# AniruddhaMandal/SS-GNN

Measured on AMD Instinct MI355X. Metric: k_subgraphs_sampled_per_sec, higher is better.
Workload: dtype int64; 1 GPU; c5_er_1m; graphs=1, columns=19999981, k=8, rows_per_gpu=1000000, global_rows=1000000, mode=sample, collate=none (single GPU)

## Files before the change

### ss-gnn_amd/csrc/ugs_kernels.hip

```cpp
#include "ugs_device.h"
#include <cstdlib>

#define UGS_ALIGNED16 __attribute__((aligned(16)))

#ifdef UGS_STAMPS
__device__ unsigned long long ugs_stamp_buffer[32];
#define ST_ ws.ST
#define STAMP_DECL unsigned long long st_t0 = 0
#define STAMP_BEGIN() do { __builtin_amdgcn_sched_barrier(0); st_t0 = __builtin_amdgcn_s_memtime(); __builtin_amdgcn_sched_barrier(0); } while (0)
#define STAMP_END(i) do { __builtin_amdgcn_sched_barrier(0); const unsigned long long t1_ = __builtin_amdgcn_s_memtime(); \
    if ((threadIdx.x & 63) == 0) { atomicAdd(&ST_[i], t1_ - st_t0); atomicAdd(&ST_[16 + (i)], 1ull); } st_t0 = __builtin_amdgcn_s_memtime(); __builtin_amdgcn_sched_barrier(0); } while (0)
#define STAMP_SUB_BEGIN() __builtin_amdgcn_sched_barrier(0); const unsigned long long sti_ = __builtin_amdgcn_s_memtime(); __builtin_amdgcn_sched_barrier(0)
#define STAMP_SUB_END_OF(parent, i) do { __builtin_amdgcn_sched_barrier(0); const unsigned long long t1_ = __builtin_amdgcn_s_memtime(); \
    if ((threadIdx.x & 63) == 0) { atomicAdd(&ST_[i], t1_ - sti_); atomicAdd(&ST_[parent], sti_ - t1_); atomicAdd(&ST_[16 + (i)], 1ull); } __builtin_amdgcn_sched_barrier(0); } while (0)
#define STAMP_SUB_END(i) STAMP_SUB_END_OF(2, i)
#else
#define STAMP_DECL
#define STAMP_SUB_BEGIN() do {} while (0)
#define STAMP_SUB_END(i) do {} while (0)
#define STAMP_SUB_END_OF(parent, i) do {} while (0)
#define STAMP_BEGIN() do {} while (0)
#define STAMP_END(i) do {} while (0)
#endif

// ... 864 lines not shown
    }
    return fm;
}

#define UGS_NO_ENTRY make_int2(-1, -1)
template <int GS, class SP, bool ADD, bool STG, bool GUARD = true, bool SON = false>
__device__ __forceinline__ bool scan_chunk(const Work<SP> &ws, const Grp<GS> &g, uint32_t v, uint32_t root_vi, uint32_t size, uint32_t &c,
                                           uint32_t &hcount, uint32_t &ecount, StageCtx &sc, int2 e, uint32_t p) {
    const uint32_t w = (uint32_t)e.x;
    const bool cand = e.y >= (int)root_vi;
    uint32_t slot = hash_slot(w, ws.hmask);
    const uint32_t step = hash_step(w);
    bool in_s = false;
    if constexpr (GS == 64 && sizeof(typename SP::TW) == 4) {
        if (ADD) {
            if constexpr (GUARD) { if (hcount + (uint32_t)__popcll(__ballot(cand)) > ws.hlimit) return false; }
            uint32_t seen = kKeyMask;
            STAMP_SUB_BEGIN();
            slot = probe_insert_lds(ws.HK, ws.hmask, slot, step, w, seen, e.y, root_vi);
            STAMP_SUB_END_OF(1, 6);
            const uint64_t insm = __ballot(seen == kEmpty);
            const uint64_t im = __ballot((int)seen < -1);
            const uint64_t dupm = __ballot((int)seen >= (int)kFresh);
            SP::sync();
            uint64_t fm = insm;
            if (__builtin_expect(dupm != 0ull, 0)) fm = first_of_repeated(g, w, insm, dupm);
            if (__builtin_amdgcn_inverse_ballot_w64(insm)) ws.HK[slot] = w;
            ecount += __builtin_amdgcn_inverse_ballot_w64(im) ? (w == v ? 1u : 2u) : 0u;
            if constexpr (STG) stage_hits_mask<SON>(sc, g, im, w, p, size);
            const uint32_t nnew = (uint32_t)__popcll(fm);
            if constexpr (GUARD) { if (c + nnew > ws.cap) return false; }
            if (__builtin_amdgcn_inverse_ballot_w64(fm)) ws.D[c + g.below(fm)] = w;
            c += nnew;
            hcount += nnew;
            SP::sync();
        } else {
            uint32_t seen = kEmpty;
            probe_find_lds(ws.HK, ws.hmask, slot, step, w, seen, e.y, root_vi);
            const uint64_t im = __ballot((int)seen < -1);
            ecount += __builtin_amdgcn_inverse_ballot_w64(im) ? (w == v ? 1u : 2u) : 0u;
            if constexpr (STG) stage_hits_mask<SON>(sc, g, im, w, p, size);
        }
        return true;
    } else
    if (ADD) {
        if constexpr (GUARD) { if (hcount + (uint32_t)__popcll(g.ballot(cand)) > ws.hlimit) return false; }
        uint32_t seen = kKeyMask;
        STAMP_SUB_BEGIN();
        if constexpr (sizeof(typename SP::TW) == 4) {
            slot = probe_insert_lds_v(reinterpret_cast<uint32_t *>(ws.HK), ws.hmask, slot, step, w, seen, e.y, root_vi);
        } else
        if (cand) {
            for (uint32_t it = 0; it <= ws.hmask; ++it) {
                seen = atomicCAS(&ws.HK[slot], kEmpty, w | kFresh);
                if (seen == kEmpty || (seen & kKeyMask) == w) break;
                slot = (slot + step) & ws.hmask;
            }
        }
        STAMP_SUB_END_OF(1, 6);
        const bool inserted = seen == kEmpty;
        in_s = (seen & (kKeyMask | kInS)) == (w | kInS);
        const bool fresh_dup = (seen & (kKeyMask | kFresh)) == (w | kFresh);
        SP::sync();
        bool first = inserted;
        uint64_t dupm = g.ballot(fresh_dup);
        while (dupm) {
            const int li = __ffsll((long long)dupm) - 1;
            const uint32_t wi = g.bcast(w, li);
            const bool mine = cand && w == wi;
            const uint64_t grp = g.ballot(mine);
            if (mine) first = g.lane == (__ffsll((long long)grp) - 1);
            dupm &= ~grp;
        }
        if (inserted) ws.HK[slot] = w;
        if constexpr (GS == 64) ecount += in_s ? (w == v ? 1u : 2u) : 0u;
        else
        {
            const uint64_t im = g.ballot(in_s), sm = g.ballot(w == v);
            ecount += 2u * (uint32_t)__popcll(im & ~sm) + (uint32_t)__popcll(im & sm);
        }
        if constexpr (STG) { if (sc.on) stage_hits<GS>(sc, g, in_s, w, p, size); }
        const uint64_t fm = g.ballot(first);
        const uint32_t nnew = (uint32_t)__popcll(fm);
        if constexpr (GUARD) { if (c + nnew > ws.cap) return false; }
        if (first) ws.D[c + g.below(fm)] = w;
        c += nnew;
        hcount += nnew;
        SP::sync();
    } else {
        uint32_t seen = kEmpty;
        if constexpr (sizeof(typename SP::TW) == 4) {
            probe_find_lds_v(reinterpret_cast<const uint32_t *>(ws.HK), ws.hmask, slot, step, w, seen, e.y, root_vi);
        } else
        if (cand) {
            for (uint32_t it = 0; it <= ws.hmask; ++it) {
                seen = ws.HK[slot];
                if (seen == kEmpty || (seen & kKeyMask) == w) break;
                slot = (slot + step) & ws.hmask;
            }
        }
        in_s = (seen & (kKeyMask | kInS)) == (w | kInS);
        if constexpr (GS == 64) ecount += in_s ? (w == v ? 1u : 2u) : 0u;
        else
        {
            const uint64_t im = g.ballot(in_s), sm = g.ballot(w == v);
            ecount += 2u * (uint32_t)__popcll(im & ~sm) + (uint32_t)__popcll(im & sm);
        }
        if constexpr (STG) { if (sc.on) stage_hits<GS>(sc, g, in_s, w, p, size); }
    }
    return true;
}

constexpr uint32_t kNoMember = 0xFFFFFFFEu;
__device__ __forceinline__ uint32_t last_row_members(const Grp<64> &g, const uint32_t *SV, uint32_t size) {
    return (uint32_t)g.lane < size ? SV[g.lane & (UGS_KMAX - 1)] : kNoMember;
}
template <bool SON>
__device__ __forceinline__ void scan_chunk_last(const Grp<64> &g, uint32_t v, uint32_t size, uint32_t &ecount, StageCtx &sc,
                                                uint32_t w, uint32_t p, uint32_t members) {
    uint64_t im = 0ull;
#pragma unroll
    for (int j = 0; j < 8; ++j) im |= __ballot(w == (uint32_t)__builtin_amdgcn_readlane((int)members, j));
    if (__builtin_expect(size > 8u, 0)) {
        for (uint32_t j = 8; j < size; j += 4) {
#pragma unroll
            for (uint32_t u = 0; u < 4; ++u) im |= __ballot(w == (uint32_t)__builtin_amdgcn_readlane((int)members, (int)(j + u)));
        }
    }
    ecount += __builtin_amdgcn_inverse_ballot_w64(im) ? (w == v ? 1u : 2u) : 0u;
    stage_hits_mask<SON>(sc, g, im, w, p, size);
}

template <int GS, class SP, bool ADD, bool STG, bool LAST = false>
__device__ __forceinline__ bool scan_row(const Work<SP> &ws, const Grp<GS> &g, const int2 *adj, uint32_t v,
                                         uint32_t root_vi, uint32_t size, uint32_t &c, uint32_t &hcount,
                                         uint32_t &ecount, uint32_t r0, uint32_t r1, StageCtx &sc, const uint32_t *SV = nullptr) {
    if constexpr (LAST) {
        static_assert(GS == 64 && STG && !ADD, "the compare form of the last row: one walk per wave, LDS tiers");
        const uint32_t members = last_row_members(g, SV, size);
        for (uint32_t base = r0; base < r1; base += 64) {
            const uint32_t p = base + (uint32_t)g.lane;
            int2 e = UGS_NO_ENTRY;
            if (p < r1) e = adj[p];
            scan_chunk_last<false>(g, v, size, ecount, sc, (uint32_t)e.x, p, members);
        }
        return true;
    }
    for (uint32_t base = r0; base < r1; base += GS) {
        const uint32_t p = base + (uint32_t)g.lane;
        int2 e = UGS_NO_ENTRY;
        if (p < r1) e = adj[p];
        if (!scan_chunk<GS, SP, ADD, STG>(ws, g, v, root_vi, size, c, hcount, ecount, sc, e, p)) return false;
    }
    return true;
}

__device__ __forceinline__ int2 prow_entry(const UgsPlanDev &P, int64_t vrow, int lane) {
    const uint32_t off = (((uint32_t)vrow << P.prow_shift) + (uint32_t)lane) << 3;
    return *reinterpret_cast<const int2 *>(reinterpret_cast<const char *>(P.prow) + off);
}
__device__ __forceinline__ int2 load_prow(const UgsPlanDev &P, int64_t vrow, int lane) {
    int2 e = make_int2(0, 0);
    if (lane < P.prow_first) e = prow_entry(P, vrow, lane);
    return e;
}

template <class SP, bool ADD, bool STG, bool SON = false, bool LAST = false>
__device__ __forceinline__ bool scan_prow(const Work<SP> &ws, const Grp<64> &g, const UgsPlanDev &P, uint32_t v,
                                          uint32_t root_vi, uint32_t size, uint32_t &c, uint32_t &hcount,
                                          uint32_t &ecount, int2 e0, int64_t vrow, StageCtx &sc, const uint32_t *SV = nullptr) {
    const uint32_t deg = g.bcast((uint32_t)e0.x, 0);
    const uint32_t start = g.bcast((uint32_t)e0.y, 0);
    const uint32_t inl = (1u << P.prow_shift) - 1u;
    const uint32_t n0 = deg < inl ? deg : inl;
    if (n0 >= (uint32_t)P.prow_first) {
        if (g.lane >= P.prow_first && g.lane <= (int)n0) e0 = prow_entry(P, vrow, g.lane);
    }
    if ((uint32_t)(g.lane - 1) >= n0) e0 = UGS_NO_ENTRY;
    if constexpr (LAST) {
        static_assert(STG && !ADD, "the compare form of the last row: one walk per wave, LDS tiers");
        const uint32_t members = last_row_members(g, SV, size);
        if (n0) scan_chunk_last<SON>(g, v, size, ecount, sc, (uint32_t)e0.x, start + (uint32_t)g.lane - 1u, members);
        if (__builtin_expect(deg > inl, 0)) {
            const uint32_t r1 = start + deg;
            for (uint32_t base = start + inl; base < r1; base += 64) {
                const uint32_t p = base + (uint32_t)g.lane;
                int2 e = UGS_NO_ENTRY;
                if (p < r1) e = P.adj[p];
                scan_chunk_last<SON>(g, v, size, ecount, sc, (uint32_t)e.x, p, members);
            }
        }
        return true;
    }
    uint32_t n0a = n0, n0b = n0;
    asm volatile("" : "+s"(n0a));
    asm volatile("" : "+s"(n0b));
    if constexpr (ADD) {
        if (__builtin_expect(hcount + deg <= ws.hlimit && c + deg <= ws.cap, 1)) {
            if (n0a) scan_chunk<64, SP, true, STG, false, SON>(ws, g, v, root_vi, size, c, hcount, ecount, sc, e0, start + (uint32_t)g.lane - 1u);
            if (__builtin_expect(deg > inl, 0)) {
                const uint32_t r1 = start + deg;
                for (uint32_t base = start + inl; base < r1; base += 64) {
                    const uint32_t p = base + (uint32_t)g.lane;
                    int2 e = UGS_NO_ENTRY;
                    if (p < r1) e = P.adj[p];
                    scan_chunk<64, SP, true, STG, false, SON>(ws, g, v, root_vi, size, c, hcount, ecount, sc, e, p);
                }
            }
            return true;
        }
    }
    if (n0b && !scan_chunk<64, SP, ADD, STG, true, SON>(ws, g, v, root_vi, size, c, hcount, ecount, sc, e0, start + (uint32_t)g.lane - 1u)) return false;
    if (__builtin_expect(deg > inl, 0)) {
        const uint32_t r1 = start + deg;
        for (uint32_t base = start + inl; base < r1; base += 64) {
            const uint32_t p = base + (uint32_t)g.lane;
            int2 e = UGS_NO_ENTRY;
            if (p < r1) e = P.adj[p];
            if (!scan_chunk<64, SP, ADD, STG, true, SON>(ws, g, v, root_vi, size, c, hcount, ecount, sc, e, p)) return false;
        }
    }
    return true;
}

constexpr uint32_t kFlushFast = 8u;
#define UGS_ROR_LT(R) "v_sub_co_u32_dpp %1, vcc, %2, %2 row_ror:" #R " row_mask:0xf bank_mask:0xf\n\ts_nop 1\n\tv_addc_co_u32_e32 %0, vcc, 0, %0, vcc\n\t"
template <int N> __device__ __forceinline__ uint32_t ror_count_less(uint32_t key) {
    static_assert(N == 7 || N == 15, "half a DPP row or all of it");
    uint32_t n, diff;
    if constexpr (N == 7)
        asm("v_mov_b32 %0, 0\n\ts_nop 0\n\t" UGS_ROR_LT(1) UGS_ROR_LT(2) UGS_ROR_LT(3) UGS_ROR_LT(4) UGS_ROR_LT(5) UGS_ROR_LT(6) UGS_ROR_LT(7)
            : "=&v"(n), "=&v"(diff) : "v"(key) : "vcc");
    else
        asm("v_mov_b32 %0, 0\n\ts_nop 0\n\t" UGS_ROR_LT(1) UGS_ROR_LT(2) UGS_ROR_LT(3) UGS_ROR_LT(4) UGS_ROR_LT(5) UGS_ROR_LT(6) UGS_ROR_LT(7)
            UGS_ROR_LT(8) UGS_ROR_LT(9) UGS_ROR_LT(10) UGS_ROR_LT(11) UGS_ROR_LT(12) UGS_ROR_LT(13) UGS_ROR_LT(14) UGS_ROR_LT(15)
            : "=&v"(n), "=&v"(diff) : "v"(key) : "vcc");
    return n;
}
#undef UGS_ROR_LT
__device__ __forceinline__ uint32_t flush_hit_lane(uint32_t ne, uint32_t lane) { return ne <= kFlushFast ? (lane & 7u) : lane; }
__device__ __forceinline__ bool flush_has_hit(uint32_t ne, uint32_t lane) {
    return ne <= kFlushFast ? (lane < 16u && (lane & 7u) < ne) : lane < ne;
}

__device__ __forceinline__ void stage_flush(uint32_t ne, const Grp<64> &g, const uint32_t *SV, uint32_t k, uint4 en, uint32_t ecol, uint2 *out) {
    const uint32_t lane = (uint32_t)g.lane;
    uint32_t ei = 0u;
    if (k <= 8u) {
        const uint4 s0 = reinterpret_cast<const uint4 *>(SV)[0], s1 = reinterpret_cast<const uint4 *>(SV)[1];
        ei = (s1.w == en.y) ? 7u : ei; ei = (s1.z == en.y) ? 6u : ei; ei = (s1.y == en.y) ? 5u : ei; ei = (s1.x == en.y) ? 4u : ei;
        ei = (s0.w == en.y) ? 3u : ei; ei = (s0.z == en.y) ? 2u : ei; ei = (s0.y == en.y) ? 1u : ei; ei = (s0.x == en.y) ? 0u : ei;
    } else {
        for (uint32_t j = 0; j < k; ++j) ei = (SV[j] == en.y) ? j : ei;
    }
    const uint32_t es = en.z;
    if (__builtin_expect(ne <= kFlushFast, 1)) {
        const bool have = lane < 16u && (lane & 7u) < ne;
        if (__builtin_expect(!g.any(have && ei == es), 1)) {
            const uint32_t col = have ? ecol : 0xFFFFFFFFu;
            const uint32_t cr = ror_count_less<7>(col);
            const bool fwd = lane < 8u;
            const uint32_t src = fwd ? es : ei, dst = fwd ? ei : es;
            const uint32_t key = have ? src * 8u + cr : 0xFFFFFFFFu;
            const uint32_t rank = ror_count_less<15>(key);
            if (have) out[rank] = make_uint2(ecol, src | (dst << 8));
            return;
        }
    }
    const bool mine = lane < ne;
    uint32_t cr = 0u;
    const uint32_t ecol_s = mine ? ecol : 0xFFFFFFFFu;
    if (g.any(mine && ei == es)) {
        for (uint32_t t = 0; t < ne; t += 4) {
#pragma unroll
            for (uint32_t u = 0; u < 4; ++u) {
                const uint32_t ct = g.bcast(ecol_s, (int)((t + u) & 63u));
                cr += (ct < ecol || (ct == ecol && t + u < lane)) ? 1u : 0u;
            }
        }
    } else {
        for (uint32_t t = 0; t < ne; t += 4) {
#pragma unroll
            for (uint32_t u = 0; u < 4; ++u) cr += g.bcast(ecol_s, (int)((t + u) & 63u)) < ecol ? 1u : 0u;
        }
    }
    const bool mirror = mine && ei != es;
    const uint32_t ka = es * UGS_STAGE_ENTRIES + cr, kb = ei * UGS_STAGE_ENTRIES + cr;
    const uint32_t kk = (ka << 16) | kb;
    uint32_t ra = 0u, rb = 0u;
    const uint32_t kk_s = mine ? kk : 0xFFFFFFFFu;
    for (uint32_t t = 0; t < ne; t += 4) {
#pragma unroll
        for (uint32_t u = 0; u < 4; ++u) {
            const uint32_t kt = g.bcast(kk_s, (int)((t + u) & 63u));
            const uint32_t kat = kt >> 16, kbt = ((kt >> 21) == ((kt >> 5) & 0x7FFu)) ? 0xFFFFu : (kt & 0xFFFFu);
            ra += (kat < ka ? 1u : 0u) + (kbt < ka ? 1u : 0u);
            rb += (kat < kb ? 1u : 0u) + (kbt < kb ? 1u : 0u);
        }
    }
    if (mine) out[ra] = make_uint2(ecol, es | (ei << 8));
    if (mirror) out[rb] = make_uint2(ecol, ei | (es << 8));
}

template <int GS, class SP, int MAXPER, bool PAD, bool SEEDS = false, bool UNI = false>
__device__ __forceinline__ bool do_walk(const Work<SP> &ws, const Grp<GS> &g_, const UgsWalkArgs &a, int64_t row_rel,
                                        uint32_t *SV , uint4 *EL ,
                                        uint32_t *nedges_out = nullptr ) {

    static_assert(!PAD || GS == 64, "padded rows are read by a whole wave");
    static_assert(!UNI || (PAD && !SEEDS && sizeof(typename SP::TW) == 4), "UNI: one graph, one seed, padded rows, staging on");
    const Grp<GS> &g = g_;
    constexpr bool STG = GS == 64 && sizeof(typename SP::TW) == 4;
    StageCtx sc;
    sc.EL = EL; sc.ne = 0u; sc.on = STG && a.stage != nullptr && EL != nullptr; sc.onm = 0ull;
    if constexpr (UNI) { sc.on = true; sc.onm = ~0ull; }
    else if constexpr (STG) {
        uint32_t on32 = g.uni(sc.on ? 1u : 0u);
        asm volatile("" : "+s"(on32));
        sc.onm = 0ull - (uint64_t)on32;
    }
    const UgsPlanDev &P = a.plan;
    const int64_t row = a.row_begin + row_rel;
    int64_t gi, i;
    if (UNI || P.num_graphs == 1) { gi = 0; i = row; }
    else { gi = row / a.m; i = row - gi * a.m; }
    const UgsGraphDesc gd = P.graphs[gi];
    const int k = a.k;
    int64_t *out = a.nodes + row_rel * k;
    if (nedges_out) *nedges_out = 0u;
    if (gd.level < 0) {
        for (int j = g.lane; j < k; j += GS) out[j] = -1;
        if (g.lane == 0) a.counts[row_rel] = 0;
        return true;
    }
    STAMP_DECL;
    STAMP_BEGIN();
    Rng rng;
    uint64_t seed_base;
    if constexpr (SEEDS) seed_base = a.seeds[gi];
    else seed_base = a.seed_ptr ? *a.seed_ptr : a.seed64;
    rng.init(seed_base + (uint64_t)i * 0x9e3779b97f4a7c15ull);
    uint32_t root_vi, root_v;
    uint32_t j = 0;
    double u = 0.0;
    UgsRootRec rr{};
    int2 vr = make_int2(0, 0);
    if (gd.level == 0) {
        j = mod64_root(rng.next(), (uint32_t)gd.n);
        u = (double)rng.next() * 0x1p-64;
        rr = P.roots[gd.vbase + j];
    } else {
        const uint32_t idx = mod64_root(rng.next(), (uint32_t)gd.n_viable);
        vr = P.viable[gd.viable_base + idx];
    }
    __builtin_amdgcn_sched_barrier(0);
    {
        uint4 *H4 = reinterpret_cast<uint4 *>(ws.HK);
        const uint32_t n4 = (ws.hmask + 1u) >> 2;
        for (uint32_t s = g.lane; s < n4; s += GS) H4[s] = make_uint4(kEmpty, kEmpty, kEmpty, kEmpty);
    }
    if (gd.level == 0) {
        const bool self = u < rr.prob;
        root_vi = g.uni(self ? j : (uint32_t)rr.alias);
        root_v = g.uni((uint32_t)(self ? rr.v_self : rr.v_alias));
    } else {
        root_vi = g.uni((uint32_t)vr.x);
        root_v = g.uni((uint32_t)vr.y);
    }
    uint32_t r0 = 0, r1 = 0;
    int2 e0 = make_int2(0, 0);
    uint32_t v = root_v;
    if constexpr (PAD) e0 = load_prow(P, gd.vbase + v, g.lane);
    else { r0 = g.uni((uint32_t)P.rowptr[gd.rbase + v]); r1 = g.uni((uint32_t)P.rowptr[gd.rbase + v + 1]); }
    SP::sync();
    if (g.lane == 0) { ws.HK[hash_slot(root_v, ws.hmask)] = root_v | kInS; SV[0] = root_v; }
    SP::sync();
    uint32_t size = 1, c = 0, hcount = 1, ecount = 0;
    int nvalid = 0;
    STAMP_END(0);
    const bool root_only = STG && k == 1;
    bool last_row = root_only;
    for (int step = 0; !root_only; ++step) {
        Grp<GS> g = g_;
        if constexpr (GS == 64) asm volatile("" : "+v"(g.lane));
#ifdef UGS_PAD
        {
            uint32_t pad_;
#if UGS_PAD == 1
#define UGS_PAD1 asm volatile("s_mov_b32 %0, 0" : "=s"(pad_));
#elif UGS_PAD == 2
#define UGS_PAD1 asm volatile("s_mov_b32 %0, 0x12345678" : "=s"(pad_));
#elif UGS_PAD == 3
#define UGS_PAD1 asm volatile("v_mov_b32_e32 %0, 0" : "=v"(pad_));
#elif UGS_PAD == 4
#define UGS_PAD1 asm volatile("v_mov_b32_e64 %0, 0" : "=v"(pad_));
#elif UGS_PAD == 5
#define UGS_PAD1 asm volatile("s_cmp_eq_u32 0, 0\ns_cbranch_scc0 ugs_pad_%=\nugs_pad_%=:" : "=s"(pad_) : : "scc");
#elif UGS_PAD == 6
#define UGS_PAD1 asm volatile("s_branch ugs_pad_%=\nugs_pad_%=:" : "=s"(pad_));
#elif UGS_PAD == 7
#define UGS_PAD1 asm volatile("s_nop 0" : "=s"(pad_));
#elif UGS_PAD == 8
#define UGS_PAD1 asm volatile("s_nop 1" : "=s"(pad_));
#else
#define UGS_PAD1 asm volatile("s_waitcnt lgkmcnt(0)" : "=s"(pad_));
#endif
#define UGS_PAD8 UGS_PAD1 UGS_PAD1 UGS_PAD1 UGS_PAD1 UGS_PAD1 UGS_PAD1 UGS_PAD1 UGS_PAD1
            UGS_PAD8 UGS_PAD8 UGS_PAD8 UGS_PAD8 UGS_PAD8 UGS_PAD8 UGS_PAD8 UGS_PAD8
#undef UGS_PAD8
#undef UGS_PAD1
        }
#endif
        bool ok;
        if constexpr (STG) {
            if constexpr (PAD) ok = scan_prow<SP, true, STG, UNI>(ws, g, P, v, root_vi, size, c, hcount, ecount, e0, gd.vbase + v, sc);
            else ok = scan_row<GS, SP, true, STG>(ws, g, P.adj, v, root_vi, size, c, hcount, ecount, r0, r1, sc);
            STAMP_END(1);
            if (!ok) return false;
            if (c == 0) break;
        } else {
            if (step < k - 1) {
                if constexpr (PAD) ok = scan_prow<SP, true, STG, UNI>(ws, g, P, v, root_vi, size, c, hcount, ecount, e0, gd.vbase + v, sc);
                else ok = scan_row<GS, SP, true, STG>(ws, g, P.adj, v, root_vi, size, c, hcount, ecount, r0, r1, sc);
            } else {
                if constexpr (PAD) ok = scan_prow<SP, false, STG, UNI>(ws, g, P, v, root_vi, size, c, hcount, ecount, e0, gd.vbase + v, sc);
                else ok = scan_row<GS, SP, false, STG>(ws, g, P.adj, v, root_vi, size, c, hcount, ecount, r0, r1, sc);
            }
            STAMP_END(1);
            if (!ok) return false;
            if (step >= k - 1 || c == 0) break;
        }
        const uint32_t rsel = g.uni(mod64_by<sizeof(typename SP::TW) == 4, sizeof(typename SP::TW) == 4 && GS == 64>(rng.next(), c));
        STAMP_END(4);
        const Pick pick = select_any<GS, MAXPER>(ws, g, c, rsel, nvalid);
        const uint32_t w = pick.w;
        if constexpr (PAD) {
            e0 = load_prow(P, gd.vbase + w, g.lane);
        } else {
            r0 = (uint32_t)P.rowptr[gd.rbase + w];
            r1 = (uint32_t)P.rowptr[gd.rbase + w + 1];
            r0 = g.uni(r0); r1 = g.uni(r1);
        }
        STAMP_END(2);
        if constexpr (STG) {
            if (size + 1u == (uint32_t)k) {
                SV[size] = w;
                size += 1;
                v = w;
                SP::sync();
                last_row = true;
                break;
            }
        }
        uint32_t q = pick.q;
        if constexpr (sizeof(typename SP::TW) != 4) {
            for (uint32_t t0 = 0; t0 < c && q == c; t0 += 4 * GS) {
                uint32_t x[4];
#pragma unroll
                for (int u = 0; u < 4; ++u) { const uint32_t t = t0 + u * GS + g.lane; x[u] = (t < c) ? ws.D[t] : kEmpty; }
#pragma unroll
                for (int u = 0; u < 4; ++u) {
                    const uint64_t mk = g.ballot(x[u] == w);
                    if (mk && q == c) q = t0 + u * GS + (uint32_t)(__ffsll((long long)mk) - 1);
                }
            }
        }
        STAMP_END(7);
        for (uint32_t t0 = q; t0 + 1 < c; t0 += 4 * GS) {
            uint32_t x[4];
            if constexpr (sizeof(typename SP::TW) == 4) {
#pragma unroll
                for (int u = 0; u < 4; ++u) x[u] = ws.D[t0 + u * GS + g.lane + 1];
                SP::sync();
                {
                    const uint32_t tb = t0 + (uint32_t)g.lane;
                    constexpr uint32_t last = (uint32_t)(MAXPER * GS) - 1u;
#pragma unroll
                    for (int u = 0; u < 4; ++u) {
                        const uint32_t lim4 = (last - (uint32_t)(u * GS)) * 4u, tb4 = tb * 4u;
                        *reinterpret_cast<uint32_t *>(reinterpret_cast<char *>(ws.D + u * GS) + (tb4 < lim4 ? tb4 : lim4)) = x[u];
                    }
                }
            } else {
#pragma unroll
                for (int u = 0; u < 4; ++u) { const uint32_t t = t0 + u * GS + g.lane; x[u] = (t + 1 < c) ? ws.D[t + 1] : 0u; }
                SP::sync();
#pragma unroll
                for (int u = 0; u < 4; ++u) { const uint32_t t = t0 + u * GS + g.lane; if (t + 1 < c) ws.D[t] = x[u]; }
            }
            SP::sync();
        }
        {
            int keep = 0;
            if constexpr (sizeof(typename SP::TW) == 4) {
                if constexpr (GS == 64) keep = chain_index_below_lanes(q + 1u, g_.chain); else
                keep = chain_index_below<nst_of(MAXPER * GS)>(q + 1u);
                keep = keep < nvalid ? keep : nvalid;
            } else {
                while (keep < nvalid && d_chain.B[keep] <= q) ++keep;
            }
            nvalid = keep;
        }
        c -= 1;
        STAMP_END(8);
        {
            const uint32_t step = hash_step(w);
            if constexpr (GS == 64 && sizeof(typename SP::TW) == 4) {
                uint32_t ls;
                asm("v_mul_u32_u24 %0, %1, %2" : "=v"(ls) : "s"(step), "v"(g.lane));
                uint32_t s = (hash_slot(w, ws.hmask) + ls) & ws.hmask;
                const uint32_t addr = (uint32_t)(uintptr_t)ws.HK + (s << 2);
                uint32_t t;
                uint64_t saved, found;
                asm volatile(
                    "s_mov_b64 %[sv], exec\n"
                    "ds_read_b32 %[t], %[addr]\n"
                    "s_waitcnt lgkmcnt(0)\n"
                    "v_cmpx_eq_u32 %[w], %[t]\n"
                    "ds_write_b32 %[addr], %[wf]\n"
                    "s_mov_b64 %[fd], exec\n"
                    "s_mov_b64 exec, %[sv]\n"
                    : [t] "=&v"(t), [sv] "=&s"(saved), [fd] "=&s"(found)
                    : [addr] "v"(addr), [w] "s"(w), [wf] "v"(w | kInS)
                    : "vcc", "memory");
                if (__builtin_expect(found == 0ull, 0)) {
                    bool hit = false;
                    for (uint32_t it = GS; !g.any(hit) && it <= ws.hmask; it += GS) {
                        s = (s + GS * step) & ws.hmask;
                        hit = ws.HK[s] == w;
                    }
                    if (hit) ws.HK[s] = w | kInS;
                }
            } else {
            uint32_t s = (hash_slot(w, ws.hmask) + (uint32_t)g.lane * step) & ws.hmask;
            bool hit = ws.HK[s] == w;
            for (uint32_t it = GS; __builtin_expect(!g.any(hit), 0) && it <= ws.hmask; it += GS) {
                s = (s + GS * step) & ws.hmask;
                hit = ws.HK[s] == w;
            }
            if (hit) ws.HK[s] = w | kInS;
            }
            if constexpr (GS == 64) SV[size] = w;
            else
            if (g.lane == 0) SV[size] = w;
        }
        size += 1;
        v = w;
        SP::sync();
        STAMP_END(3);
    }
    if constexpr (STG) {
        if (last_row) {
            if constexpr (PAD) (void)scan_prow<SP, false, STG, UNI, true>(ws, g, P, v, root_vi, size, c, hcount, ecount, e0, gd.vbase + v, sc, SV);
            else (void)scan_row<GS, SP, false, STG, true>(ws, g, P.adj, v, root_vi, size, c, hcount, ecount, r0, r1, sc, SV);
            STAMP_END(1);
        }
    }
    if constexpr (GS == 64) ecount = g.last(g.prefix_incl(ecount));
    const uint32_t nedges = (size == (uint32_t)k) ? ecount : 0u;
    bool flush = false;
    uint4 en = make_uint4(0u, 0u, 0u, 0u);
    uint32_t ecol = 0u;
    if constexpr (STG) {
        flush = sc.on && nedges != 0u && sc.ne <= UGS_STAGE_ENTRIES;
        if (flush && flush_has_hit(sc.ne, (uint32_t)g.lane)) { en = sc.EL[flush_hit_lane(sc.ne, (uint32_t)g.lane)]; ecol = (uint32_t)P.adjf[en.x].y; }
    }
    const int64_t off = gd.node_lo + a.extra_node_off;
    for (int j = g.lane; j < k; j += GS) out[j] = (j < (int)size) ? (int64_t)SV[j] + off : (int64_t)-1;
    if (g.lane == 0) a.counts[row_rel] = nedges | (flush ? UGS_COUNT_STAGED : 0u);
    if (nedges_out) *nedges_out = nedges;
    if (UNI || a.stage) {
        if constexpr (STG) { if (flush) stage_flush(sc.ne, g, SV, (uint32_t)k, en, ecol, a.stage + row_rel * UGS_STAGE_ITEMS); }
        if (g.lane == 0 && !flush && nedges != 0u) a.ulist[atomicAdd(a.ucount, 1u)] = row_rel;
    }
    STAMP_END(5);
    return true;
}

template <int CAP> struct TierCfg {
    static constexpr int NSTAGE = nst_of(CAP);
    static constexpr int ORDW = (int)(((ord_words_before(NSTAGE) + 1u) / 2u + 3u) & ~3u);
    static constexpr int TI = tier_index(CAP);
    static constexpr int BCAP_A = tbl_words(CAP);
    static constexpr int HS = CAP <= 32 ? 64 : (TI == 0 ? 128 : (TI == 1 ? 512 : (TI == 2 ? 1024 : (TI <= 4 ? 2048 : 4096))));
    static constexpr int HLIMIT = (TI == 1 || TI == 2 || TI == 4) ? HS / 8 * 7 : HS / 4 * 3;
    static_assert(CAP <= 64 || BCAP_A * 4 >= 127 * 16, "mates2_by_table keeps 16 bytes per bucket of the 127-bucket stage in TBL");
    static_assert(CAP == UGS_SMALL_CAP ? HLIMIT == UGS_SMALL_HASH_LIMIT : (HLIMIT == UGS_TIER_HASH_LIMIT[TI] && CAP == UGS_TIER_CAP[TI]),
                  "host tier logic (choose_tier) relies on these limits");
    static constexpr int ELW = CAP > 64 ? 4 * UGS_STAGE_ENTRIES : 0;
    static constexpr int WORDS = CAP  + ORDW + BCAP_A  + HS  + UGS_KMAX  + ELW;
};

template <int GS, int CAP, int BLOCK, bool PAD, bool SEEDS = false, bool UNI = false>
__global__ __launch_bounds__(BLOCK, CAP <= 32 ? 4 : ((CAP > 64 && CAP <= 512) ? 5 : (CAP == 704 ? 3 : (CAP <= 64 || CAP == 1024 || CAP == 1408 ? 2 : 1)))) void ugs_walk_lds(UgsWalkArgs a) {
    using Cfg = TierCfg<CAP>;
    constexpr int GROUPS = BLOCK / GS;
    __shared__ __attribute__((aligned(16))) uint32_t lds[GROUPS * Cfg::WORDS];
    Grp<GS> g;
    g.init();
    if constexpr (GS == 64) g.chain = chain_lane_const<Cfg::NSTAGE>(g.lane);
    const int gib = (int)threadIdx.x / GS;
    uint32_t *base = lds + gib * Cfg::WORDS;
    Work<LdsSpace> ws;
    ws.D = base;
    ws.ORD = reinterpret_cast<uint16_t *>(ws.D + CAP);
    ws.AUX = nullptr;
    ws.TBL = ws.D + CAP + Cfg::ORDW;
    ws.HK = ws.TBL + Cfg::BCAP_A;
    uint32_t *SV = ws.HK + Cfg::HS;
    uint4 *EL = Cfg::ELW ? reinterpret_cast<uint4 *>(SV + UGS_KMAX) : nullptr;
    ws.cap = CAP;
    ws.hmask = Cfg::HS - 1;
    ws.hlimit = Cfg::HLIMIT;
#ifdef UGS_STAMPS
    __shared__ unsigned long long stamps[32];
    if (threadIdx.x < 32) stamps[threadIdx.x] = 0ull;
    __syncthreads();
    ws.ST = stamps;
    struct Flush { unsigned long long *st; __device__ ~Flush() { __syncthreads(); if (threadIdx.x < 32) atomicAdd(&ugs_stamp_buffer[threadIdx.x], st[threadIdx.x]); } } flush_{stamps};
#endif
    const int64_t total = (!UNI && a.in_list) ? (int64_t)*a.in_count : a.row_count;
    const int64_t ngroups = (int64_t)gridDim.x * GROUPS;
    if (a.work_next) {
        auto chunk_for = [&](int64_t left) -> int64_t { return left > 8 * ngroups ? 4 : (left > 2 * ngroups ? 2 : 1); };
        const int64_t first = chunk_for(total);
        int64_t it = ((int64_t)blockIdx.x * GROUPS + gib) * first, end = it + first;
        while (it < total) {
            if (end > total) end = total;
            for (; it < end; ++it) {
                const int64_t row_rel = (!UNI && a.in_list) ? a.in_list[it] : it;
                if (!do_walk<GS, LdsSpace, (CAP + GS - 1) / GS, PAD, SEEDS, UNI>(ws, g, a, row_rel, SV, EL)) {
                    if (g.lane == 0 && a.ovf_list) { uint32_t pos = atomicAdd(a.ovf_count, 1u); a.ovf_list[pos] = row_rel; }
                }
            }
            const int64_t chunk = chunk_for(total - it);
            unsigned long long nxt = 0ull;
            if (g.lane == 0) nxt = atomicAdd(a.work_next, (unsigned long long)chunk);
            const uint32_t lo = g.bcast((uint32_t)nxt, 0), hi = g.bcast((uint32_t)(nxt >> 32), 0);
            it = ngroups * first + (int64_t)(((unsigned long long)hi << 32) | lo);
            end = it + chunk;
        }
        return;
    }
    if constexpr (GS == 8 || GS == 16) {
        if (a.wsum) {
            constexpr int RPW = 64 / GS;
            __shared__ uint32_t wave_sum[BLOCK / 64];
            for (int64_t it0 = (int64_t)blockIdx.x * GROUPS; it0 < total; it0 += ngroups) {
                const int64_t it = it0 + gib;
                uint32_t ne = 0u;
                if (it < total) (void)do_walk<GS, LdsSpace, (CAP + GS - 1) / GS, PAD, SEEDS>(ws, g, a, it, SV, EL, &ne);
                uint32_t sum = g.lane == 0 ? ne : 0u;
#pragma unroll
                for (int d = GS; d < 64; d <<= 1) sum += __shfl_xor(sum, d, 64);
                if constexpr (RPW == 8) {
                    const int64_t w0 = it0 + (int64_t)((threadIdx.x >> 6) * 8);
                    if ((threadIdx.x & 63) == 0 && w0 < total) a.wsum[w0 >> 3] = sum;
                } else {
                    if ((threadIdx.x & 63) == 0) wave_sum[threadIdx.x >> 6] = sum;
                    __syncthreads();
                    if (threadIdx.x < GROUPS / 8) {
                        const int64_t r0 = it0 + (int64_t)threadIdx.x * 8;
                        if (r0 < total) a.wsum[r0 >> 3] = wave_sum[2 * threadIdx.x] + wave_sum[2 * threadIdx.x + 1];
                    }
                    __syncthreads();
                }
            }
            return;
        }
    }
    for (int64_t it = (int64_t)blockIdx.x * GROUPS + gib; it < total; it += ngroups) {
        const int64_t row_rel = (!UNI && a.in_list) ? a.in_list[it] : it;
        if (!do_walk<GS, LdsSpace, (CAP + GS - 1) / GS, PAD, SEEDS, UNI>(ws, g, a, row_rel, SV, EL)) {
            if (g.lane == 0 && a.ovf_list) { uint32_t pos = atomicAdd(a.ovf_count, 1u); a.ovf_list[pos] = row_rel; }
        }
    }
}

__global__ __launch_bounds__(256) void ugs_build_prow(UgsPlanDev P, int64_t num_vertices, int2 *prow, int shift) {
    const int64_t idx = (int64_t)blockIdx.x * 256 + threadIdx.x;
    const int64_t R = idx >> shift;
    if (R >= num_vertices) return;
    const int l = (int)(idx & ((1 << shift) - 1));
    int64_t lo = 0, hi = P.num_graphs - 1;
    while (lo < hi) {
        const int64_t mid = (lo + hi + 1) >> 1;
        if (P.graphs[mid].vbase <= R) lo = mid; else hi = mid - 1;
    }
    const int64_t rb = P.graphs[lo].rbase, v = R - P.graphs[lo].vbase;
    const int64_t start = P.rowptr[rb + v], deg = P.rowptr[rb + v + 1] - start;
    int2 e = make_int2(0, 0);
    if (l == 0) e = make_int2((int)deg, (int)start);
    else if (l - 1 < deg) e = P.adj[start + l - 1];
    prow[idx] = e;
}

template <bool SEEDS>
__global__ __launch_bounds__(64) void ugs_walk_global(UgsWalkArgs a) {
    __shared__ uint32_t SV[UGS_KMAX];
    Grp<64> g;
    g.init();
    uint32_t *base = a.gws + (int64_t)blockIdx.x * a.gws_words_per_group;
    Work<GlbSpace> ws;
    auto al4 = [](int64_t x) { return (x + 3) & ~3ll; };
    ws.TBL = (unsigned long long *)base;
    ws.D = base + 2 * al4(a.gbcap);
    ws.ORD = ws.D + al4(a.gcap);
    ws.AUX = ws.ORD + al4(a.gpcap);
    ws.HK = ws.AUX + al4(a.gcap);
    ws.cap = (uint32_t)a.gcap;
    ws.hmask = (uint32_t)a.ghs - 1u;
    ws.hlimit = (uint32_t)a.ghs / 4u * 3u;
#ifdef UGS_STAMPS
    __shared__ unsigned long long stamps[32];
    ws.ST = stamps;
#endif
    const int64_t total = a.in_list ? (int64_t)*a.in_count : a.row_count;
    for (int64_t it = blockIdx.x; it < total; it += gridDim.x) {
        const int64_t row_rel = a.in_list ? a.in_list[it] : it;
        if (!do_walk<64, GlbSpace, 0, false, SEEDS>(ws, g, a, row_rel, SV, nullptr)) {
            if (g.lane == 0 && a.ovf_list) { uint32_t pos = atomicAdd(a.ovf_count, 1u); a.ovf_list[pos] = row_rel; }
        }
    }
}

constexpr int kScanBlock = 256, kScanPer = 8, kScanTile = kScanBlock * kScanPer;

__device__ __forceinline__ int64_t block_excl_scan(int64_t x, int64_t *total, int64_t *sh ) {
    const int lane = threadIdx.x & 63, wv = threadIdx.x >> 6;
    long long incl = x;
#pragma unroll
    for (int d = 1; d < 64; d <<= 1) { long long y = __shfl_up(incl, d, 64); if (lane >= d) incl += y; }
    if (lane == 63) sh[wv] = incl;
    __syncthreads();
    int64_t woff = 0, tot = 0;
#pragma unroll
    for (int i = 0; i < kScanBlock / 64; ++i) { if (i < wv) woff += sh[i]; tot += sh[i]; }
    __syncthreads();
    *total = tot;
    return woff + incl - x;
}

__global__ __launch_bounds__(kScanBlock) void ugs_scan_partials(const uint32_t *counts, int64_t rows, int64_t *block_sums) {
    __shared__ int64_t sh[kScanBlock / 64];
    const int64_t base = (int64_t)blockIdx.x * kScanTile + (int64_t)threadIdx.x * kScanPer;
    int64_t s = 0;
#pragma unroll
    for (int j = 0; j < kScanPer; ++j) if (base + j < rows) s += counts[base + j] & ~UGS_COUNT_STAGED;
    int64_t tot;
    block_excl_scan(s, &tot, sh);
    if (threadIdx.x == 0) block_sums[blockIdx.x] = tot;
}

__global__ __launch_bounds__(kScanBlock) void ugs_scan_block_sums(int64_t *block_sums, int64_t nblocks) {
    __shared__ int64_t sh[kScanBlock / 64];
    int64_t carry = 0;
    for (int64_t base = 0; base < nblocks; base += kScanBlock) {
        const int64_t idx = base + threadIdx.x;
        int64_t x = idx < nblocks ? block_sums[idx] : 0, tot;
        int64_t ex = block_excl_scan(x, &tot, sh);
        if (idx < nblocks) block_sums[idx] = carry + ex;
        carry += tot;
    }
}

struct ScanSignal { int64_t *h_total; uint32_t *h_flag; uint32_t epoch; };
__device__ __forceinline__ void scan_signal(const ScanSignal &sg, int64_t total) {
    if (sg.h_total) { *sg.h_total = total; __threadfence_system(); *(volatile uint32_t *)sg.h_flag = sg.epoch; }
}

__global__ __launch_bounds__(kScanBlock) void ugs_scan_final(const uint32_t *counts, int64_t rows, const int64_t *block_offs,
                                                             int64_t *edge_ptr, ScanSignal sg) {
    __shared__ int64_t sh[kScanBlock / 64];
    const int64_t base = (int64_t)blockIdx.x * kScanTile + (int64_t)threadIdx.x * kScanPer;
    uint32_t v[kScanPer];
    int64_t s = 0;
#pragma unroll
    for (int j = 0; j < kScanPer; ++j) { v[j] = (base + j < rows) ? (counts[base + j] & ~UGS_COUNT_STAGED) : 0u; s += v[j]; }
    int64_t tot;
    int64_t ex = block_excl_scan(s, &tot, sh) + (block_offs ? block_offs[blockIdx.x] : 0);
#pragma unroll
    for (int j = 0; j < kScanPer; ++j) { if (base + j < rows) edge_ptr[base + j] = ex; ex += v[j]; }
    if (rows - 1 >= base && rows - 1 < base + kScanPer) { edge_ptr[rows] = ex; scan_signal(sg, ex); }
}

__global__ __launch_bounds__(kScanBlock) void ugs_scan_final_sum(const uint32_t *counts, int64_t rows, const int64_t *tile_sums,
                                                                 int64_t *edge_ptr, ScanSignal sg) {
    __shared__ int64_t sh[kScanBlock / 64];
    int64_t before = 0, front;
    for (int64_t i = threadIdx.x; i < (int64_t)blockIdx.x; i += kScanBlock) before += tile_sums[i];
    block_excl_scan(before, &front, sh);
    const int64_t base = (int64_t)blockIdx.x * kScanTile + (int64_t)threadIdx.x * kScanPer;
    uint32_t v[kScanPer];
    int64_t s = 0;
#pragma unroll
    for (int j = 0; j < kScanPer; ++j) { v[j] = (base + j < rows) ? (counts[base + j] & ~UGS_COUNT_STAGED) : 0u; s += v[j]; }
    int64_t tot;
    int64_t ex = block_excl_scan(s, &tot, sh) + front;
#pragma unroll
    for (int j = 0; j < kScanPer; ++j) { if (base + j < rows) edge_ptr[base + j] = ex; ex += v[j]; }
    if (rows - 1 >= base && rows - 1 < base + kScanPer) { edge_ptr[rows] = ex; scan_signal(sg, ex); }
}

constexpr int kScanWide = 1024;
__global__ __launch_bounds__(kScanWide) void ugs_scan_small(const uint32_t *counts, int64_t rows, int64_t *edge_ptr, ScanSignal sg) {
    __shared__ int64_t sh[kScanWide / 64];
    const int lane = threadIdx.x & 63, wv = threadIdx.x >> 6;
    int64_t carry = 0;
    for (int64_t tile = 0; tile < rows; tile += (int64_t)kScanWide * kScanPer) {
        const int64_t base = tile + (int64_t)threadIdx.x * kScanPer;
        uint32_t v[kScanPer];
        int64_t s = 0;
#pragma unroll
        for (int j = 0; j < kScanPer; ++j) { v[j] = (base + j < rows) ? (counts[base + j] & ~UGS_COUNT_STAGED) : 0u; s += v[j]; }
        long long incl = s;
#pragma unroll
        for (int d = 1; d < 64; d <<= 1) { long long y = __shfl_up(incl, d, 64); if (lane >= d) incl += y; }
        if (lane == 63) sh[wv] = incl;
        __syncthreads();
        int64_t woff = 0, tot = 0;
#pragma unroll
        for (int i = 0; i < kScanWide / 64; ++i) { if (i < wv) woff += sh[i]; tot += sh[i]; }
        __syncthreads();
        int64_t ex = carry + woff + incl - s;
#pragma unroll
        for (int j = 0; j < kScanPer; ++j) { if (base + j < rows) edge_ptr[base + j] = ex; ex += v[j]; }
        carry += tot;
    }
    if (threadIdx.x == 0) { edge_ptr[rows] = carry; scan_signal(sg, carry); }
}

template <int GS>
__device__ __forceinline__ void fill_row(const UgsFillArgs &a, const int64_t *rowptr, const int2 *adjf, const Grp<GS> &g, const UgsGraphDesc &gd, int64_t row_rel, int64_t i,
                                         int64_t e0, const int64_t *nrow, const uint32_t *SVsrc, uint32_t *SV, uint32_t *PS, int64_t *R0) {
    const int k = a.k;
    const int64_t off = gd.node_lo + a.extra_node_off;
    LdsSpace::sync();
    for (int j = g.lane; j < k; j += GS) {
        const uint32_t u = nrow ? (uint32_t)(nrow[j] - off) : SVsrc[j];
        const int64_t r0 = rowptr[gd.rbase + u], r1 = rowptr[gd.rbase + u + 1];
        SV[j] = u;
        R0[j] = r0;
        PS[j + 1] = (uint32_t)(r1 - r0);
    }
    LdsSpace::sync();
    if (g.lane == 0) { uint32_t acc = 0; PS[0] = 0; for (int j = 1; j <= k; ++j) { acc += PS[j]; PS[j] = acc; } }
    LdsSpace::sync();
    const uint32_t T = PS[k];
    int64_t w_off = e0;
    if (k <= 8) {
        uint32_t ps[9], sv[8];
#pragma unroll
        for (int t = 0; t < 8; ++t) { sv[t] = (t < k) ? SV[t] : 0xFFFFFFFEu ; ps[t] = (t < k) ? PS[t] : 0xFFFFFFFFu; }
        ps[8] = 0xFFFFFFFFu;
        for (uint32_t cb = 0; cb < T; cb += 4 * GS) {
            uint32_t wv[4];
            int jj[4], ec[4];
#pragma unroll
            for (int u = 0; u < 4; ++u) {
                const uint32_t e = cb + u * GS + g.lane;
                wv[u] = kEmpty; jj[u] = 0; ec[u] = 0;
                if (e < T) {
                    int j = 0;
#pragma unroll
                    for (int t = 1; t < 8; ++t) j += (ps[t] <= e) ? 1 : 0;
                    uint32_t base_e = ps[0];
#pragma unroll
                    for (int t = 1; t < 8; ++t) base_e = (j == t) ? ps[t] : base_e;
                    jj[u] = j;
                    const int2 nb = adjf[R0[j] + (int64_t)(e - base_e)];
                    wv[u] = (uint32_t)nb.x;
                    ec[u] = nb.y;
                }
            }
#pragma unroll
            for (int u = 0; u < 4; ++u) {
                if (cb + u * GS >= T) break;
                int l = -1;
#pragma unroll
                for (int t = 7; t >= 0; --t) l = (sv[t] == wv[u]) ? t : l;
                const uint64_t mk = g.ballot(l >= 0);
                const int64_t pos = w_off + g.below(mk);
                if (l >= 0 && pos < a.ld) {
                    const int j = jj[u];
                    int64_t uf, vf;
                    if (a.mode == 0) { uf = j; vf = l; }
                    else if (a.mode == 1) { uf = i * k + j; vf = i * k + l; }
                    else if (a.mode == 3) { uf = row_rel * k + j; vf = row_rel * k + l; }
                    else { uf = (int64_t)SV[j] + off; vf = (int64_t)SV[l] + off; }
                    a.edge_index[pos] = uf;
                    a.edge_index[a.ld + pos] = vf;
                    a.edge_src[pos] = (int64_t)ec[u];
                }
                w_off += __popcll(mk);
            }
        }
        return;
    }
    for (uint32_t cb = 0; cb < T; cb += 4 * GS) {
        uint32_t wv[4];
        int jj[4], ec[4];
#pragma unroll
        for (int u = 0; u < 4; ++u) {
            const uint32_t e = cb + u * GS + g.lane;
            wv[u] = kEmpty; jj[u] = 0; ec[u] = 0;
            if (e < T) {
                int j = 0;
                for (int t = 1; t < k; ++t) j += (PS[t] <= e) ? 1 : 0;
                jj[u] = j;
                const int2 nb = adjf[R0[j] + (int64_t)(e - PS[j])];
                wv[u] = (uint32_t)nb.x;
                ec[u] = nb.y;
            }
        }
#pragma unroll
        for (int u = 0; u < 4; ++u) {
            if (cb + u * GS >= T) break;
            int l = -1;
            if (wv[u] != kEmpty) { for (int t = 0; t < k; ++t) if (SV[t] == wv[u]) { l = t; break; } }
            const uint64_t mk = g.ballot(l >= 0);
            const int64_t pos = w_off + g.below(mk);
            if (l >= 0 && pos < a.ld) {
                const int j = jj[u];
                int64_t uf, vf;
                if (a.mode == 0) { uf = j; vf = l; }
                else if (a.mode == 1) { uf = i * k + j; vf = i * k + l; }
// ... 324 lines not shown
```

Before: 226.0 million k-subgraphs/s.

## Precompute per-chunk RNG draws and root picks across wave lanes

For the single-graph uniform path, each wave now computes all random draws for up to four rows of a work chunk in parallel. Each lane owns one (row, draw) pair and one lane per row also resolves the root via the alias or viable table. The walk then reads its draws and root with readlane instead of stepping the xorshift serially and doing the root lookup on the critical path. This takes the serial RNG chain and root-table latency off each walk. In exchange every lane runs a short redundant xorshift loop, there is a new code path, and the path only applies when the number of draws is at most 16.

```diff
diff --git a/ss-gnn_amd/csrc/ugs_kernels.hip b/ss-gnn_amd/csrc/ugs_kernels.hip
--- a/ss-gnn_amd/csrc/ugs_kernels.hip
+++ b/ss-gnn_amd/csrc/ugs_kernels.hip
@@ -1190,10 +1190,48 @@
     if (mirror) out[rb] = make_uint2(ecol, ei | (es << 8));
 }
 
-template <int GS, class SP, int MAXPER, bool PAD, bool SEEDS = false, bool UNI = false>
+struct ChunkDraws {
+    uint32_t lo = 0u, hi = 0u;
+    int base = 0;
+};
+__device__ __forceinline__ void chunk_draws(const UgsWalkArgs &a, int64_t row0 , int nd,
+                                            int wl , ChunkDraws &cd) {
+    const UgsPlanDev &P = a.plan;
+    const UgsGraphDesc gd = P.graphs[0];
+    const uint64_t seed_base = a.seed_ptr ? *a.seed_ptr : a.seed64;
+    const uint32_t r = (uint32_t)wl >> 4, j = (uint32_t)wl & 15u;
+    uint64_t s = seed_base + (uint64_t)(row0 + (int64_t)r) * 0x9e3779b97f4a7c15ull;
+    s = s ? s : 1ull;
+    uint64_t keep = 0ull;
+    for (uint32_t t = 0; t < (uint32_t)nd; ++t) {
+        s ^= s >> 12; s ^= s << 25; s ^= s >> 27;
+        keep = t == j ? s : keep;
+    }
+    const uint64_t x = keep * 2685821657736338717ull;
+    cd.lo = (uint32_t)x; cd.hi = (uint32_t)(x >> 32);
+    if (gd.level == 0) {
+        const uint32_t lo2 = (uint32_t)__builtin_amdgcn_update_dpp(0, (int)cd.lo, 0x101, 0xf, 0xf, false);
+        const uint32_t hi2 = (uint32_t)__builtin_amdgcn_update_dpp(0, (int)cd.hi, 0x101, 0xf, 0xf, false);
+        const uint32_t idx = mod64_root(x, (uint32_t)gd.n);
+        const double u = (double)(((uint64_t)hi2 << 32) | lo2) * 0x1p-64;
+        UgsRootRec rr{};
+        if (j == 0u) rr = P.roots[gd.vbase + idx];
+        const bool self = u < rr.prob;
+        if (j == 0u) { cd.lo = self ? idx : (uint32_t)rr.alias; cd.hi = (uint32_t)(self ? rr.v_self : rr.v_alias); }
+    } else {
+        const uint32_t idx = mod64_root(x, (uint32_t)gd.n_viable);
+        int2 vr = make_int2(0, 0);
+        if (j == 0u) vr = P.viable[gd.viable_base + idx];
+        if (j == 0u) { cd.lo = (uint32_t)vr.x; cd.hi = (uint32_t)vr.y; }
+    }
+}
+
+template <int GS, class SP, int MAXPER, bool PAD, bool SEEDS = false, bool UNI = false, bool CHK = false>
 __device__ __forceinline__ bool do_walk(const Work<SP> &ws, const Grp<GS> &g_, const UgsWalkArgs &a, int64_t row_rel,
                                         uint32_t *SV , uint4 *EL ,
-                                        uint32_t *nedges_out = nullptr ) {
+                                        uint32_t *nedges_out = nullptr ,
+                                        const ChunkDraws &cd = ChunkDraws{}) {
+    static_assert(!CHK || UNI, "chunk draws: the UNI instantiation's dynamic loop only");
 
     static_assert(!PAD || GS == 64, "padded rows are read by a whole wave");
     static_assert(!UNI || (PAD && !SEEDS && sizeof(typename SP::TW) == 4), "UNI: one graph, one seed, padded rows, staging on");
@@ -1216,7 +1254,7 @@
     const int k = a.k;
     int64_t *out = a.nodes + row_rel * k;
     if (nedges_out) *nedges_out = 0u;
-    if (gd.level < 0) {
+    if (!CHK && gd.level < 0) {
         for (int j = g.lane; j < k; j += GS) out[j] = -1;
         if (g.lane == 0) a.counts[row_rel] = 0;
         return true;
@@ -1224,15 +1262,25 @@
     STAMP_DECL;
     STAMP_BEGIN();
     Rng rng;
-    uint64_t seed_base;
-    if constexpr (SEEDS) seed_base = a.seeds[gi];
-    else seed_base = a.seed_ptr ? *a.seed_ptr : a.seed64;
-    rng.init(seed_base + (uint64_t)i * 0x9e3779b97f4a7c15ull);
+    if constexpr (CHK) rng.s = 0ull;
+    else {
+        uint64_t seed_base;
+        if constexpr (SEEDS) seed_base = a.seeds[gi];
+        else seed_base = a.seed_ptr ? *a.seed_ptr : a.seed64;
+        rng.init(seed_base + (uint64_t)i * 0x9e3779b97f4a7c15ull);
+    }
     uint32_t root_vi, root_v;
     uint32_t j = 0;
     double u = 0.0;
     UgsRootRec rr{};
     int2 vr = make_int2(0, 0);
+    uint32_t r0 = 0, r1 = 0;
+    int2 e0 = make_int2(0, 0);
+    if constexpr (CHK) {
+        root_vi = (uint32_t)__builtin_amdgcn_readlane((int)cd.lo, cd.base & 48);
+        root_v = (uint32_t)__builtin_amdgcn_readlane((int)cd.hi, cd.base & 48);
+        e0 = load_prow(P, gd.vbase + root_v, g.lane);
+    } else
     if (gd.level == 0) {
         j = mod64_root(rng.next(), (uint32_t)gd.n);
         u = (double)rng.next() * 0x1p-64;
@@ -1247,6 +1295,8 @@
         const uint32_t n4 = (ws.hmask + 1u) >> 2;
         for (uint32_t s = g.lane; s < n4; s += GS) H4[s] = make_uint4(kEmpty, kEmpty, kEmpty, kEmpty);
     }
+    if constexpr (CHK) {
+    } else
     if (gd.level == 0) {
         const bool self = u < rr.prob;
         root_vi = g.uni(self ? j : (uint32_t)rr.alias);
@@ -1255,9 +1305,9 @@
         root_vi = g.uni((uint32_t)vr.x);
         root_v = g.uni((uint32_t)vr.y);
     }
-    uint32_t r0 = 0, r1 = 0;
-    int2 e0 = make_int2(0, 0);
     uint32_t v = root_v;
+    if constexpr (CHK) {
+    } else
     if constexpr (PAD) e0 = load_prow(P, gd.vbase + v, g.lane);
     else { r0 = g.uni((uint32_t)P.rowptr[gd.rbase + v]); r1 = g.uni((uint32_t)P.rowptr[gd.rbase + v + 1]); }
     SP::sync();
@@ -1318,7 +1368,12 @@
             if (!ok) return false;
             if (step >= k - 1 || c == 0) break;
         }
-        const uint32_t rsel = g.uni(mod64_by<sizeof(typename SP::TW) == 4, sizeof(typename SP::TW) == 4 && GS == 64>(rng.next(), c));
+        uint64_t x;
+        if constexpr (CHK) {
+            const int src = cd.base + step;
+            x = ((uint64_t)(uint32_t)__builtin_amdgcn_readlane((int)cd.hi, src) << 32) | (uint64_t)(uint32_t)__builtin_amdgcn_readlane((int)cd.lo, src);
+        } else x = rng.next();
+        const uint32_t rsel = g.uni(mod64_by<sizeof(typename SP::TW) == 4, sizeof(typename SP::TW) == 4 && GS == 64>(x, c));
         STAMP_END(4);
         const Pick pick = select_any<GS, MAXPER>(ws, g, c, rsel, nvalid);
         const uint32_t w = pick.w;
@@ -1510,6 +1565,33 @@
     const int64_t total = (!UNI && a.in_list) ? (int64_t)*a.in_count : a.row_count;
     const int64_t ngroups = (int64_t)gridDim.x * GROUPS;
     if (a.work_next) {
+        if constexpr (UNI) {
+            const int level = a.plan.graphs[0].level;
+            const int nd = level == 0 ? a.k + 1 : a.k;
+            if (level >= 0 && nd <= 16) {
+                const int draw0 = nd - a.k + 1;
+                auto chunk_for = [&](int64_t left) -> int64_t { return left > 8 * ngroups ? 4 : (left > 2 * ngroups ? 2 : 1); };
+                const int64_t first = chunk_for(total);
+                int64_t it = ((int64_t)blockIdx.x * GROUPS + gib) * first, end = it + first;
+                while (it < total) {
+                    if (end > total) end = total;
+                    ChunkDraws cd;
+                    chunk_draws(a, a.row_begin + it, nd, g.lane, cd);
+                    for (cd.base = draw0; it < end; ++it, cd.base += 16) {
+                        if (!do_walk<GS, LdsSpace, (CAP + GS - 1) / GS, PAD, SEEDS, UNI, true>(ws, g, a, it, SV, EL, nullptr, cd)) {
+                            if (g.lane == 0 && a.ovf_list) { uint32_t pos = atomicAdd(a.ovf_count, 1u); a.ovf_list[pos] = it; }
+                        }
+                    }
+                    const int64_t chunk = chunk_for(total - it);
+                    unsigned long long nxt = 0ull;
+                    if (g.lane == 0) nxt = atomicAdd(a.work_next, (unsigned long long)chunk);
+                    const uint32_t lo = g.bcast((uint32_t)nxt, 0), hi = g.bcast((uint32_t)(nxt >> 32), 0);
+                    it = ngroups * first + (int64_t)(((unsigned long long)hi << 32) | lo);
+                    end = it + chunk;
+                }
+                return;
+            }
+        }
         auto chunk_for = [&](int64_t left) -> int64_t { return left > 8 * ngroups ? 4 : (left > 2 * ngroups ? 2 : 1); };
         const int64_t first = chunk_for(total);
         int64_t it = ((int64_t)blockIdx.x * GROUPS + gib) * first, end = it + first;
```

Result: no change. 227.9 million k-subgraphs/s, median of 6 (+0.8%).
